# suhrig/arriba

Measured on AMD Instinct MI355X. Metric: chimeric reads/s end-to-end (BAM->fusions.tsv), synthetic, higher is better.
Workload: dtype int32

## Files before the change

### arriba_amd/csrc/device/agpu_ingest.hip

```cpp
#include <hip/hip_runtime.h>
#include <algorithm>
#include <cstring>
#include <string>
#include <vector>
#include <rocprim/rocprim.hpp>
#include "agpu_context.hpp"
#include "ingest_core.hpp"
#include "device_utils.hpp"
#include "shard_host.hpp"
#include "crc32_core.hpp"
#include "inflate_fast_core.hpp"

using namespace agpu;
namespace agpu { extern thread_local bool g_inside_ingest_finish; }

namespace {

const int BLOCK = 256;
inline unsigned int grid_for(uint64_t n, int block = BLOCK) { return (unsigned int) ((n + block - 1) / block); }

enum { IC_ACTIVE = 0, IC_MAPPED_READS = 1, IC_MISSING_HI = 2, IC_BROKEN = 3, IC_MALFORMED = 4, IC_CHIMERIC = 5, IC_COLLISION = 6, IC_MISMATCH = 7, IC_UNSORTED = 8, IC_MAX_NAME = 9,
       IC_MAX_READ_LENGTH = 10, IC_STRAND_COUNT = 11, IC_STRAND_MATCHING = 12, IC_RUNS_UNSORTED = 13, IC_QNAME_COMMA = 14, IC_COUNT = 16 };

#define HIP_CHECK(call) do { hipError_t e_ = (call); if (e_ != hipSuccess) { set_last_error(std::string(#call) + ": " + hipGetErrorString(e_)); return AGPU_ERR_DEVICE; } } while (0)
// ... 280 lines not shown
	block_tally(tally.chimeric, &counters[IC_CHIMERIC], &sums[1]);
}


__device__ FragmentName name_of(const IngestStream& in, const uint32_t* group_first, uint32_t ref, Rec& storage) {
	storage = load_record(in, group_first[ref >> 1]);
	return fragment_name(storage, hit_index_of(in, group_first[ref >> 1], storage), ref & 1);
}

__global__ void name_order_check_kernel(IngestStream in, const uint32_t* group_first, const uint32_t* order, uint64_t n, uint32_t* counters) {
	__shared__ uint32_t block_max;
	if (threadIdx.x == 0) block_max = 0;
	__syncthreads();
	const uint64_t i = blockIdx.x * (uint64_t) BLOCK + threadIdx.x;
	if (i < n) {
		Rec storage_a, storage_b;
		const FragmentName mine = name_of(in, group_first, order[i], storage_a);
		atomicMax(&block_max, name_length(mine));
		if (i > 0) {
			const FragmentName before = name_of(in, group_first, order[i - 1], storage_b);
			if (compare_names(before, mine) >= 0) atomicOr(&counters[IC_UNSORTED], 1u);
		}
	}
	__syncthreads();
	if (threadIdx.x == 0 && block_max) atomicMax(&counters[IC_MAX_NAME], block_max);
}

__global__ void run_itd_order_kernel(IngestStream in, const uint32_t* group_first, const uint8_t* valid, uint32_t first_group, uint32_t n_groups, uint32_t* counters) {
	const uint32_t g = first_group + blockIdx.x * BLOCK + threadIdx.x;
	if (g >= n_groups || g == 0 || !valid[2 * (size_t) (g - 1) + 1]) return;
	Rec storage_a, storage_b;
	const FragmentName mine = name_of(in, group_first, 2 * g, storage_b);
	const FragmentName before = name_of(in, group_first, 2 * (g - 1) + 1, storage_a);
	if (compare_names(before, mine) >= 0) atomicOr(&counters[IC_RUNS_UNSORTED], 1u);
}

__global__ void name_chunk_kernel(IngestStream in, const uint32_t* group_first, const uint32_t* order, uint64_t n, uint32_t chunk, uint64_t* keys) {
	const uint64_t i = blockIdx.x * (uint64_t) BLOCK + threadIdx.x;
	if (i >= n) return;
	Rec storage;
	keys[i] = name_chunk(name_of(in, group_first, order[i], storage), chunk);
}


__global__ void fragment_layout_kernel(IngestStream in, const uint32_t* group_first, const uint32_t* order, uint64_t n, const FragmentSizes* sizes, const uint32_t* qname_run ,
                                       uint32_t* cigar_words, uint32_t* sequence_bytes, uint32_t* name_lengths, uint32_t* new_group) {
	const uint64_t i = blockIdx.x * (uint64_t) BLOCK + threadIdx.x;
	if (i > n) return;
	if (i == n) { cigar_words[i] = 0; sequence_bytes[i] = 0; name_lengths[i] = 0; return; }
	const uint32_t ref = order[i];
	const FragmentSizes mine = sizes[ref];
	cigar_words[i] = mine.cigar_words; sequence_bytes[i] = mine.sequence_bytes; name_lengths[i] = mine.name_length;
	uint32_t differs = 0;
	if (i > 0 && qname_run != nullptr) differs = qname_run[ref >> 1] != qname_run[order[i - 1] >> 1];
	else if (i > 0) {
		const Rec a = load_record(in, group_first[ref >> 1]), b = load_record(in, group_first[order[i - 1] >> 1]);
		const uint32_t length = qname_length(a);
		differs = length != qname_length(b);
		for (uint32_t k = 0; k < length && !differs; ++k) differs = a.name[k] != b.name[k];
	}
	new_group[i] = differs;
}

__global__ void __launch_bounds__(BLOCK) AGPU_PACK_OCCUPANCY fragment_pack_kernel(IngestStream in, const uint32_t* group_first, const uint32_t* order, uint64_t n, const FragmentPlan* plain, const TandemPlan* itd,
                                                              const uint64_t* cigar_base, const uint64_t* sequence_base, const uint64_t* name_base, const uint32_t* group_id, PackTarget out, uint32_t* counters) {
	__shared__ uint32_t block_max;
	if (threadIdx.x == 0) block_max = 0;
	__syncthreads();
	const uint64_t i = blockIdx.x * (uint64_t) BLOCK + threadIdx.x;
	if (i == n) out.name_offset[n] = name_base[n];
	if (i < n) {
		const uint32_t ref = order[i], g = ref >> 1;
		const bool is_itd = ref & 1;
		Fragment3 f;
		normalize_plan(in, is_itd ? itd[g].plan : plain[g], is_itd ? &itd[g].tandem : nullptr, f);
		Rec storage;
		const FragmentName name = name_of(in, group_first, ref, storage);
		atomicMax(&block_max, write_fragment(in, f, name, i, cigar_base[i], sequence_base[i], name_base[i], group_id[i], out));
	}
	__syncthreads();
	if (threadIdx.x == 0 && block_max) atomicMax(&counters[IC_MAX_READ_LENGTH], block_max);
}

template <bool INFLATED> __global__ void __launch_bounds__(256) bgzf_crc_kernel(const uint8_t* raw, const agpu_bgzf_block* blocks, uint32_t n_blocks, const Crc32Tables* tables, unsigned int* mismatches) {
	__shared__ uint32_t slice[4][256];
	__shared__ uint32_t join[2][4][256];
	__shared__ uint32_t staged[4][CRC32_WAVE_LANES * (CRC32_ROUND_WORDS + 1)];
	for (uint32_t k = threadIdx.x; k < 4 * 256; k += 256) ((uint32_t*) slice)[k] = ((const uint32_t*) tables->slice)[k];
	for (uint32_t k = threadIdx.x; k < 2 * 4 * 256; k += 256) ((uint32_t*) join)[k] = ((const uint32_t*) tables->join)[k];
	const uint32_t wave = threadIdx.x / CRC32_WAVE_LANES, lane = threadIdx.x % CRC32_WAVE_LANES, b = blockIdx.x * 4 + wave;
	agpu_bgzf_block block;
	block.crc32 = 0; block.payload_size = 0; block.raw_offset = 0; block.payload_offset = 0;
	if (b < n_blocks) block = blocks[b];
	if (INFLATED) { block.raw_offset = block.stream_offset; block.payload_offset = 0; block.payload_size = block.isize; }
	const bool checked = b < n_blocks && block.crc32 != 0 && block.payload_size <= CRC32_VIRTUAL;
	const uint8_t* payload = raw + block.raw_offset + block.payload_offset;
	const uint32_t n = block.payload_size;
	uint32_t* mine = staged[wave];
	uint32_t c = 0;
	const bool by_chunks = checked && n >= 4;
	const uint32_t first_word = by_chunks ? (CRC32_VIRTUAL - n) / 4 : CRC32_VIRTUAL / 4;
	for (uint32_t round = 0; round < CRC32_WAVE_CHUNK / 4 / CRC32_ROUND_WORDS; ++round) {
		__syncthreads();
		for (uint32_t item = lane; item < CRC32_WAVE_LANES * CRC32_ROUND_WORDS; item += CRC32_WAVE_LANES) {
			const uint32_t chunk = item / CRC32_ROUND_WORDS, j = item % CRC32_ROUND_WORDS, w = chunk * (CRC32_WAVE_CHUNK / 4) + round * CRC32_ROUND_WORDS + j;
			mine[chunk * (CRC32_ROUND_WORDS + 1) + j] = w >= first_word ? crc32_virtual_word(payload, n, w) : 0u;
		}
		__syncthreads();
		for (uint32_t j = 0; j < CRC32_ROUND_WORDS; ++j) c = crc32_raw_step(slice, c, mine[lane * (CRC32_ROUND_WORDS + 1) + j]);
	}
	__syncthreads();
	mine[lane] = c;
	__syncthreads();
	if (lane % 8 == 0) { for (uint32_t i = 1; i < 8; ++i) c = crc32_apply(join[0], c) ^ mine[lane + i]; }
	__syncthreads();
	if (lane % 8 == 0) mine[lane] = c;
	__syncthreads();
	if (lane == 0 && checked) {
		for (uint32_t g = 1; g < 8; ++g) c = crc32_apply(join[1], c) ^ mine[8 * g];
		c ^= 0xFFFFFFFFu;
		if (n < 4) c = crc32_of_sliced(slice, payload, n);
		if (c != block.crc32) atomicAdd(mismatches, 1u);
	}
}

__global__ void shard_rebase_kernel(uint32_t* out, const uint32_t* in, uint64_t n, uint32_t base, const uint8_t* n_aln, uint32_t slot) {
	const uint64_t i = (uint64_t) blockIdx.x * blockDim.x + threadIdx.x;
	if (i < n) out[i] = in[i] + ((slot >= 3 || slot < n_aln[i]) ? base : 0u);
}
__global__ void shard_rebase_names_kernel(uint64_t* out, const uint64_t* in, uint64_t n, uint64_t base) {
	const uint64_t i = (uint64_t) blockIdx.x * blockDim.x + threadIdx.x;
	if (i < n) out[i] = in[i] + base;
}
__global__ void shard_add_coverage_kernel(uint32_t* windows, uint8_t* starts, uint8_t* ends, const uint32_t* part_windows, const uint8_t* part_starts, const uint8_t* part_ends, uint64_t n) {
	const uint64_t i = (uint64_t) blockIdx.x * blockDim.x + threadIdx.x;
	if (i < n) { windows[i] += part_windows[i]; starts[i] |= part_starts[i]; ends[i] |= part_ends[i]; }
}
__global__ void shard_add_counts_kernel(unsigned long long* counts, const unsigned long long* part, uint32_t n) {
	const uint32_t i = blockIdx.x * blockDim.x + threadIdx.x;
	if (i < n) counts[i] += part[i];
}

__global__ void packed_name_length_kernel(const uint64_t* name_offset, uint64_t n, uint32_t* longest) {
	const uint64_t i = blockIdx.x * (uint64_t) BLOCK + threadIdx.x;
	if (i < n) atomicMax(longest, (uint32_t) (name_offset[i + 1] - name_offset[i]));
}
__global__ void packed_name_chunk_kernel(const char* names, const uint64_t* name_offset, const uint32_t* order, uint64_t n, uint32_t chunk, uint64_t* keys) {
	const uint64_t i = blockIdx.x * (uint64_t) BLOCK + threadIdx.x;
	if (i >= n) return;
	const uint32_t row = order[i]; const uint64_t begin = name_offset[row]; const uint32_t length = (uint32_t) (name_offset[row + 1] - begin);
	uint64_t key = 0;
	for (uint32_t k = 0; k < 8; ++k) { const uint32_t at = 8 * chunk + k; key = key << 8 | (at < length ? (uint8_t) names[begin + at] : 0u); }
	keys[i] = key;
}
__global__ void packed_name_neighbours_kernel(const char* names, const uint64_t* name_offset, const uint32_t* order, uint64_t n, uint32_t* new_group, uint32_t* equal_names) {
	const uint64_t i = blockIdx.x * (uint64_t) BLOCK + threadIdx.x;
	if (i >= n) return;
	if (i == 0) { new_group[0] = 0; return; }
	const uint32_t a = order[i - 1], b = order[i]; const uint64_t begin_a = name_offset[a], begin_b = name_offset[b]; const uint32_t length_a = (uint32_t) (name_offset[a + 1] - begin_a), length_b = (uint32_t) (name_offset[b + 1] - begin_b);
	bool same = length_a == length_b;
	for (uint32_t k = 0; same && k < length_a; ++k) same = names[begin_a + k] == names[begin_b + k];
	if (same) atomicAdd(equal_names, 1u);
	uint32_t qname_a = length_a, qname_b = length_b;
	while (qname_a > 0 && names[begin_a + qname_a - 1] != ',') --qname_a;
	while (qname_b > 0 && names[begin_b + qname_b - 1] != ',') --qname_b;
	bool same_qname = qname_a == qname_b;
	for (uint32_t k = 0; same_qname && k < qname_a; ++k) same_qname = names[begin_a + k] == names[begin_b + k];
	new_group[i] = same_qname ? 0u : 1u;
}
__global__ void qname_run_flag_kernel(IngestStream in, uint64_t n_records, uint8_t* flags) {
	const uint64_t r = blockIdx.x * (uint64_t) BLOCK + threadIdx.x;
	if (r < n_records) flags[r] = starts_qname_run(in, (uint32_t) r) ? 1 : 0;
}
__global__ void qname_key_kernel(IngestStream in, const uint32_t* run_starts, uint64_t n_runs, uint64_t* keys) {
	const uint64_t k = blockIdx.x * (uint64_t) BLOCK + threadIdx.x;
	if (k < n_runs) qname_key128(load_record(in, run_starts[k]), keys[2 * k], keys[2 * k + 1]);
}
__global__ void qname_low_kernel(const uint64_t* keys, uint64_t n, uint64_t* low) { const uint64_t k = blockIdx.x * (uint64_t) BLOCK + threadIdx.x; if (k < n) low[k] = keys[2 * k]; }
__global__ void qname_equal_kernel(const uint64_t* low_sorted, const uint32_t* index_sorted, const uint64_t* keys, uint64_t n, uint32_t* equal) {
	const uint64_t k = blockIdx.x * (uint64_t) BLOCK + threadIdx.x;
	if (k > 0 && k < n && low_sorted[k] == low_sorted[k - 1] && keys[2 * (uint64_t) index_sorted[k] + 1] == keys[2 * (uint64_t) index_sorted[k - 1] + 1]) atomicAdd(equal, 1u);
}
__global__ void separate_name_key_kernel(const char* names, const uint64_t* name_offset, uint64_t n, uint64_t* keys) {
	const uint64_t i = blockIdx.x * (uint64_t) BLOCK + threadIdx.x;
	if (i >= n) return;
	const uint64_t begin = name_offset[i], size = name_offset[i + 1] - begin;
	keys[i] = qname_bytes_key((const uint8_t*) names + begin, size >= 2 ? (uint32_t) (size - 2) : 0u);
}
__global__ void separate_keep_kernel(const uint32_t* order, uint64_t n, const uint8_t* fbits, const uint8_t* n_aln, const uint8_t* abits_split_read, const uint8_t* abits_supplementary, uint32_t first_part, uint8_t* keep, uint32_t* inconsistent) {
	const uint64_t i = blockIdx.x * (uint64_t) BLOCK + threadIdx.x;
	if (i >= n) return;
	const uint32_t row = order[i];
	const bool of_pass_c = row < first_part, single_end = fbits[row] & FBIT_SINGLE_END;
	keep[i] = !(of_pass_c && single_end);
	if (of_pass_c && !single_end && n_aln[row] == 3 && ((abits_split_read[row] ^ abits_supplementary[row]) & ABIT_FIRST_IN_PAIR)) atomicAdd(inconsistent, 1u);
}
__global__ void iota_kernel(uint32_t* out, uint64_t n) { const uint64_t i = blockIdx.x * (uint64_t) BLOCK + threadIdx.x; if (i < n) out[i] = (uint32_t) i; }

__global__ void coverage_from_differences_kernel(const uint32_t* summed, const uint64_t* window_offset, uint32_t n_contigs, uint64_t n, uint32_t* counts, uint16_t* out) {
	const uint64_t i = blockIdx.x * (uint64_t) BLOCK + threadIdx.x;
	if (i >= n) return;
	uint32_t low = 0, high = n_contigs;
	while (high - low > 1) { const uint32_t middle = (low + high) / 2; if (window_offset[middle] <= i) low = middle; else high = middle; }
	const uint32_t count = summed[i + low];
	counts[i] = count;
	out[i] = count > 65535u ? (uint16_t) 65535 : (uint16_t) count;
// ... 256 lines not shown
			}
			if (w.known == w.enqueued && w.enqueued < 4 && (k == 0 || p.windows[k - 1].known > w.enqueued || (w.enqueued == 3 && p.windows[k - 1].enqueued == 4))) { TRY(window_step(ctx, w)); moved = true; }
		}
		while (!p.windows.empty() && p.windows.front().known == 4) { p.events.push_back(p.windows.front().readback); p.windows.pop_front(); moved = true; }
		if (moved) continue;
		if (!wait) break;
		for (size_t k = 0; k < p.windows.size(); ++k) if (p.windows[k].enqueued > p.windows[k].known) { HIP_CHECK(hipEventSynchronize(p.windows[k].readback)); break; }
	}
	return AGPU_OK;
}

int window_make(agpu_ctx* ctx, bool last) {
	IngestProgress& p = ctx->ingest_progress;
	const uint64_t size = ctx->ingest_stream_size, base = ctx->ingest_first_record;
	uint64_t segment_end = 0;
	if (last) segment_end = size > base ? (size - base + SEGMENT_BYTES - 1) / SEGMENT_BYTES : 0;
	else if (size > base + g_window_margin) segment_end = (size - base - g_window_margin) / SEGMENT_BYTES;
	if (!last && segment_end <= p.segments_done) return AGPU_OK;
	while (p.windows.size() + 2 > INGEST_WINDOW_RING) {
		IngestWindow& oldest = p.windows.front();
		if (oldest.enqueued > oldest.known) HIP_CHECK(hipEventSynchronize(oldest.readback));
		TRY(windows_advance(ctx, false));
		if (p.abandoned) return AGPU_OK;
	}
	IngestWindow w;
	w.avail = size; w.segment_begin = p.segments_done; w.segment_end = std::max(segment_end, p.segments_done); w.last = last; w.slot = p.next_slot; p.next_slot = (p.next_slot + 1) % INGEST_WINDOW_RING;
	if (!p.events.empty()) { w.readback = p.events.back(); p.events.pop_back(); } else HIP_CHECK(hipEventCreateWithFlags(&w.readback, hipEventDisableTiming));
	p.segments_done = w.segment_end; p.window_bytes = size; ++p.windows_made;
	if (ctx->ingest_pushes > 0) HIP_CHECK(hipStreamWaitEvent(p.work, ctx->piece_ready[(ctx->ingest_pushes - 1) % AGPU_PIECE_SLOTS], 0));
	p.windows.push_back(w);
	if (p.windows.size() == 1 || p.windows[p.windows.size() - 2].enqueued >= 1) TRY(window_step(ctx, p.windows.back()));
	return AGPU_OK;
}

int windows_after_push(agpu_ctx* ctx) {
	IngestProgress& p = ctx->ingest_progress;
	if (!p.on || p.abandoned) return AGPU_OK;
	TRY(windows_advance(ctx, false));
	if (!p.abandoned && ctx->ingest_stream_size - p.window_bytes >= g_window_bytes) TRY(window_make(ctx, false));
	return AGPU_OK;
}

void fill_pack_target(agpu_ctx* ctx, PackTarget& out) {
	out.n_aln = ctx->n_aln.as<uint8_t>(); out.fbits = ctx->fbits.as<uint8_t>(); out.group = ctx->group.as<uint32_t>();
	for (int k = 0; k < 3; ++k) {
		out.contig[k] = ctx->contig[k].as<uint16_t>(); out.start[k] = ctx->start[k].as<int32_t>(); out.end[k] = ctx->end[k].as<int32_t>(); out.abits[k] = ctx->abits[k].as<uint8_t>();
		out.cigar_offset[k] = ctx->cigar_offset[k].as<uint32_t>(); out.cigar_count[k] = ctx->cigar_count[k].as<uint16_t>();
	}
	out.cigar_pool = ctx->cigar_pool.as<uint32_t>();
	for (int k = 0; k < 2; ++k) { out.seq_offset[k] = ctx->seq_offset[k].as<uint32_t>(); out.seq_length[k] = ctx->seq_length[k].as<uint32_t>(); }
	out.seq_pool = ctx->seq_pool.as<uint8_t>(); out.name_offset = ctx->name_offset.as<uint64_t>(); out.row_name_offset = nullptr; out.names = ctx->names.as<char>();
}

struct BgzfPiece {
	const uint8_t* raw; const agpu_bgzf_block* blocks; uint32_t n_blocks;
	uint64_t raw_bytes, stream_bytes;
	uint8_t* target;
	uint8_t* spill;
	int lanes;
	unsigned long long* notes; uint32_t* note_count; int* status;
	int* verdict;
	unsigned int* counters;
	const Crc32Tables* crc_tables;
	hipEvent_t ready_before, ready;
};
int launch_bgzf_piece(agpu_ctx* ctx, hipStream_t pieces, bool deflated, const BgzfPiece& p) {
	const uint32_t n_blocks = p.n_blocks;
	if (deflated) {
		unsigned int* failures = p.counters + 1;
		if (p.lanes == -1) {
			KernelTimer timer(ctx, "bgzf_inflate_kernel", p.raw_bytes + p.stream_bytes, pieces);
			bgzf_inflate_kernel<<<n_blocks, 64, 0, pieces>>>(p.raw, p.blocks, p.target, p.spill, nullptr, p.verdict, failures);
		} else {
			{ KernelTimer timer(ctx, "bgzf_inflate_tokens_kernel", p.raw_bytes + p.stream_bytes, pieces);
			  #define TOKENS(LANES) bgzf_inflate_tokens_kernel<LANES><<<(n_blocks + LANES - 1) / LANES, LANES, 0, pieces>>>(p.raw, p.blocks, n_blocks, p.target, p.spill, p.notes, p.note_count, p.status, failures)
			  if (p.lanes == 16) TOKENS(16); else if (p.lanes == 24) TOKENS(24); else TOKENS(20);
			  #undef TOKENS
			}
			bgzf_inflate_kernel<<<n_blocks, 64, 0, pieces>>>(p.raw, p.blocks, p.target, p.spill, p.status, p.verdict, failures);
			{ KernelTimer timer(ctx, "bgzf_inflate_resolve_kernel", p.stream_bytes, pieces);
			  bgzf_inflate_resolve_kernel<<<(n_blocks + BLOCK / 64 - 1) / (BLOCK / 64), BLOCK, 0, pieces>>>(p.blocks, n_blocks, p.target, p.spill, p.notes, p.note_count, p.status); }
		}
	}
	else { KernelTimer timer(ctx, "bgzf_unwrap_kernel", p.raw_bytes + p.stream_bytes, pieces);
	  bgzf_unwrap_kernel<<<n_blocks, BLOCK, 0, pieces>>>(p.raw, p.blocks, p.target); }
	if (p.ready_before) HIP_CHECK(hipStreamWaitEvent(pieces, p.ready_before, 0));
	if (p.ready) HIP_CHECK(hipEventRecord(p.ready, pieces));
	if (p.crc_tables) {
		KernelTimer timer(ctx, "bgzf_crc_kernel", deflated ? p.stream_bytes : p.raw_bytes, pieces);
		if (deflated) bgzf_crc_kernel<true><<<(n_blocks + 3) / 4, 256, 0, pieces>>>(p.target, p.blocks, n_blocks, p.crc_tables, p.counters);
		else bgzf_crc_kernel<false><<<(n_blocks + 3) / 4, 256, 0, pieces>>>(p.raw, p.blocks, n_blocks, p.crc_tables, p.counters);
	}
	return AGPU_OK;
}
int upload_crc_tables(agpu_ctx* ctx) {
	if (ctx->scratch("ingest.crc_tables").ptr != nullptr) return AGPU_OK;
	ALLOC(ctx->scratch("ingest.crc_tables"), sizeof(Crc32Tables));
	static Crc32Tables tables; static bool made = false;
	if (!made) { crc32_make_tables(tables); made = true; }
	HIP_CHECK(hipMemcpy(ctx->scratch("ingest.crc_tables").ptr, &tables, sizeof(tables), hipMemcpyHostToDevice));
	return AGPU_OK;
}

}

int agpu::ingest_grow_stream(agpu_ctx* ctx, uint64_t needed) { return grow_stream(ctx, needed); }
int agpu::ingest_piece_pushed(agpu_ctx* ctx) {
	TRY(wait_for_previous_push(ctx));
	++ctx->ingest_pushes;
	return windows_after_push(ctx);
}

bool agpu::release_ingest_buffers(agpu_ctx* ctx) {
	bool released = ctx->ingest_stream.ptr != nullptr;
	ctx->ingest_stream.release(); for (int k = 0; k < AGPU_PIECE_SLOTS; ++k) ctx->ingest_raw[k].release();
	if (!ctx->ingest_part_of_sample) ctx->coverage_windows32.release();
	static const char* const temporary[] = { "ingest.record_offset", "ingest.keys", "ingest.keys_sorted", "ingest.record_bits", "ingest.sorted_records", "ingest.head", "ingest.group_start", "ingest.first_flags", "ingest.stream_rank", "ingest.group_first", "ingest.group_begin", "ingest.group_count", "ingest.plain_plans", "ingest.itd_plans",
		"ingest.valid", "ingest.sizes", "ingest.refs", "ingest.order", "ingest.order_keys", "ingest.order_keys_sorted", "ingest.cigar_words", "ingest.sequence_bytes", "ingest.name_lengths", "ingest.new_group", "ingest.cigar_base",
		"ingest.sequence_base", "ingest.name_base", "ingest.group_id", "ingest.qname_differs", "ingest.qname_run", "ingest.run_keys", "ingest.run_keys_sorted", "ingest.window_rocprim", "ingest.segment_first", "ingest.segment_end", "ingest.segment_end_before", "ingest.segment_count", "ingest.segment_base", "ingest.segment_mismatch", "ingest.rocprim", "ingest.coverage_summed", "ingest.hit_index",
		"sam.wave_count", "sam.wave_base", "sam.line_start", "sam.record_size", "sam.record_offset", "sam.rocprim", "sam.tool_text", "sam.tool_records",
		"bgzf.tool_raw", "bgzf.tool_blocks", "bgzf.tool_out", "bgzf.tool_notes", "bgzf.tool_note_count", "bgzf.tool_status", "bgzf.tool_verdict",
		"sortedbam.keys", "sortedbam.keys_sorted", "sortedbam.order", "sortedbam.sizes", "sortedbam.sizes_sorted", "sortedbam.end_flag", "sortedbam.out_offset", "sortedbam.block_first", "sortedbam.staging", "sortedbam.rocprim", "sortedbam.crc_tables",
		"sortedbam.ref_length", "sortedbam.interval_offset", "sortedbam.intervals", "sortedbam.ref_stats", "sortedbam.heads", "sortedbam.chunk_id", "sortedbam.chunk_key", "sortedbam.chunk_begin", "sortedbam.chunk_end", "sortedbam.chunk_key_sorted", "sortedbam.chunk_order", "sortedbam.chunk_out" };
	ctx->last_ingest_kept = false;
	for (size_t k = 0; k < sizeof(temporary) / sizeof(temporary[0]); ++k) { DeviceBuffer& buffer = ctx->scratch(temporary[k]); if (buffer.ptr != nullptr) released = true; buffer.release(); }
	return released;
}

extern "C" {

void* agpu_host_alloc(size_t bytes) {
	void* pointer = nullptr;
	if (hipHostMalloc(&pointer, bytes ? bytes : 16, hipHostMallocDefault) != hipSuccess) { set_last_error("hipHostMalloc failed"); return nullptr; }
	return pointer;
}
void agpu_host_free(void* pointer) { if (pointer) (void) hipHostFree(pointer); }

static int gather_rows_prepare(agpu_ctx* ctx, const uint32_t* fragments, uint64_t n, uint64_t* pool_sizes);

int agpu_ingest_begin(agpu_ctx* ctx, const agpu_ingest_config* config) {
	if (!ctx || !config) { set_last_error("null argument"); return AGPU_ERR_INVALID; }
	if (!ctx->have_annotation || !ctx->have_genome) { set_last_error("annotation and genome must be uploaded before the ingest"); return AGPU_ERR_INVALID; }
	if (config->n_contigs != ctx->genome.n_contigs) { set_last_error("the genome view on the device does not hold the contigs of the BAM header (upload it after the header was parsed)"); return AGPU_ERR_INVALID; }
	HIP_CHECK(hipSetDevice(ctx->device));
	hipStream_t s = ctx->stream;
	{ std::lock_guard<std::mutex> lock(ctx->profile_mutex); ctx->failed_launch.clear(); }
	if (!ctx->piece_stream) {
		int least = 0, greatest = 0;
		HIP_CHECK(hipDeviceGetStreamPriorityRange(&least, &greatest));
		const char* priorities = getenv("ARRIBA_STREAM_PRIORITIES");
		const bool pieces_first = priorities == nullptr || strcmp(priorities, "stages") != 0;
		HIP_CHECK(hipStreamCreateWithPriority(&ctx->piece_stream, hipStreamNonBlocking, pieces_first ? greatest : (least + greatest) / 2));
		HIP_CHECK(hipStreamCreateWithPriority(&ctx->piece_stream2, hipStreamNonBlocking, pieces_first ? greatest : (least + greatest) / 2));
		for (int k = 0; k < AGPU_PIECE_SLOTS; ++k) { HIP_CHECK(hipEventCreateWithFlags(&ctx->piece_copied[k], hipEventDisableTiming | hipEventBlockingSync));  HIP_CHECK(hipEventCreateWithFlags(&ctx->piece_ready[k], hipEventDisableTiming)); HIP_CHECK(hipEventCreateWithFlags(&ctx->piece_done[k], hipEventDisableTiming)); }
	}
	if (config->host_buffers > AGPU_PIECE_SLOTS) { set_last_error("agpu_ingest_config.host_buffers: at most 4"); return AGPU_ERR_INVALID; }
	if (config->role > AGPU_ROLE_SEPARATE_RNA || (config->role != AGPU_ROLE_WHOLE && config->part_of_sample)) { set_last_error("agpu_ingest_config.role: AGPU_ROLE_WHOLE, AGPU_ROLE_SEPARATE_CHIMERIC or AGPU_ROLE_SEPARATE_RNA, the latter two not as a part of a sample"); return AGPU_ERR_INVALID; }
	if (config->role == AGPU_ROLE_SEPARATE_RNA && !ctx->separate_adopted) { set_last_error("the main alignments of -c (AGPU_ROLE_SEPARATE_RNA) come behind agpu_separate_adopt of the separate chimeric file"); return AGPU_ERR_INVALID; }
	ctx->ingest_host_buffers = config->host_buffers < 2 ? 2 : config->host_buffers;
	ctx->last_ingest_kept = false; if (ctx->sibling) ctx->sibling->last_ingest_kept = false;
	ctx->ingest_n_targets = config->n_targets; ctx->ingest_first_record = config->first_record_offset; ctx->ingest_stream_size = 0; ctx->ingest_pushes = 0; ctx->ingest_deflated_pieces = false; ctx->ingest_sam = false;
	{ const char* knob = getenv("ARRIBA_VERIFY_CRC"); ctx->ingest_verify_crc = !(knob != nullptr && knob[0] == '0'); }
	ALLOC(ctx->scratch("ingest.crc_mismatches"), 8);
	if (ctx->ingest_verify_crc) TRY(upload_crc_tables(ctx));
	HIP_CHECK(hipMemsetAsync(ctx->scratch("ingest.crc_mismatches").ptr, 0, 8, s));
	ctx->ingest_external_duplicate_marking = config->external_duplicate_marking; ctx->ingest_max_itd_length = config->max_itd_length;
	ctx->ingest_role = config->role; ctx->ingest_part_of_sample = config->part_of_sample != 0 || config->role != AGPU_ROLE_WHOLE;
	if (config->role != AGPU_ROLE_SEPARATE_RNA) { ctx->separate_adopted = false; ctx->separate_block.release(); ctx->separate_keys.release(); ctx->separate_rows.release(); ctx->separate_n = 0; }
	ALLOC(ctx->ingest_tid_to_contig, std::max<size_t>(config->n_targets, 1) * 4);
	if (config->n_targets) HIP_CHECK(hipMemcpyAsync(ctx->ingest_tid_to_contig.ptr, config->tid_to_contig, (size_t) config->n_targets * 4, hipMemcpyHostToDevice, s));
	ctx->host_coverage_window_offset.assign(config->coverage_window_offset, config->coverage_window_offset + config->n_contigs + 1);
	const uint64_t windows = ctx->host_coverage_window_offset.back();
	ALLOC(ctx->coverage_window_offset, ((size_t) config->n_contigs + 1) * 8); ALLOC(ctx->coverage_windows32, std::max<uint64_t>(coverage_difference_slots(windows, config->n_contigs), 1) * 4); ALLOC(ctx->coverage_windows, std::max<uint64_t>(windows, 1) * 2);
	ALLOC(ctx->coverage_fragment_starts, std::max<uint64_t>(windows, 1)); ALLOC(ctx->coverage_fragment_ends, std::max<uint64_t>(windows, 1));
// ... 1022 lines not shown
```

### arriba_amd/csrc/device/crc32_core.hpp

```cpp
#ifndef AGPU_CRC32_CORE_HPP
#define AGPU_CRC32_CORE_HPP 1

#include "views.hpp"

namespace agpu {

const uint32_t CRC32_POLYNOMIAL = 0xEDB88320u;

AGPU_HD uint32_t crc32_table_entry(uint32_t i) {
	uint32_t c = i;
	for (int k = 0; k < 8; ++k) c = (c & 1u) ? (c >> 1) ^ CRC32_POLYNOMIAL : c >> 1;
	return c;
}
AGPU_HD uint32_t crc32_of(const uint32_t* table, const uint8_t* bytes, size_t n) {
	uint32_t c = 0xFFFFFFFFu;
	for (size_t i = 0; i < n; ++i) c = table[(c ^ bytes[i]) & 0xFFu] ^ (c >> 8);
	return c ^ 0xFFFFFFFFu;
}
AGPU_HD uint32_t gf2_matrix_times(const uint32_t* matrix, uint32_t vector) {
	uint32_t sum = 0;
	for (int k = 0; vector != 0; vector >>= 1, ++k) if (vector & 1u) sum ^= matrix[k];
	return sum;
}
AGPU_HD void gf2_matrix_square(uint32_t* square, const uint32_t* matrix) { for (int k = 0; k < 32; ++k) square[k] = gf2_matrix_times(matrix, matrix[k]); }
AGPU_HD uint32_t crc32_update_sliced(const uint32_t (*slice)[256], uint32_t c, const uint8_t* bytes, size_t n) {
	size_t i = 0;
	for (; i + 4 <= n; i += 4) {
		uint32_t word; __builtin_memcpy(&word, bytes + i, 4);
		c ^= word;
		c = slice[3][c & 0xFFu] ^ slice[2][(c >> 8) & 0xFFu] ^ slice[1][(c >> 16) & 0xFFu] ^ slice[0][c >> 24];
	}
	for (; i < n; ++i) c = slice[0][(c ^ bytes[i]) & 0xFFu] ^ (c >> 8);
	return c;
}
AGPU_HD uint32_t crc32_joined(uint32_t crc_a, uint32_t crc_b, uint64_t length_b) {
	if (length_b == 0) return crc_a;
	uint32_t even[32], odd[32];
	odd[0] = CRC32_POLYNOMIAL;
	uint32_t row = 1;
	for (int k = 1; k < 32; ++k) { odd[k] = row; row <<= 1; }
	gf2_matrix_square(even, odd);
	gf2_matrix_square(odd, even);
	do {
		gf2_matrix_square(even, odd);
		if (length_b & 1u) crc_a = gf2_matrix_times(even, crc_a);
		length_b >>= 1;
		if (length_b == 0) break;
		gf2_matrix_square(odd, even);
		if (length_b & 1u) crc_a = gf2_matrix_times(odd, crc_a);
		length_b >>= 1;
	} while (length_b != 0);
	return crc_a ^ crc_b;
}

const uint32_t CRC32_CHUNK = 256;

const int CRC32_ADVANCE_POWERS = 17;
const uint32_t CRC32_WAVE_CHUNK = 1024, CRC32_WAVE_LANES = 64, CRC32_VIRTUAL = CRC32_WAVE_CHUNK * CRC32_WAVE_LANES, CRC32_ROUND_WORDS = 16;
struct Crc32Tables { uint32_t slice[4][256]; uint32_t advance[CRC32_ADVANCE_POWERS][32]; uint32_t join[2][4][256]; };
AGPU_HD uint32_t crc32_apply(const uint32_t (*op)[256], uint32_t c) { return op[0][c & 0xFFu] ^ op[1][(c >> 8) & 0xFFu] ^ op[2][(c >> 16) & 0xFFu] ^ op[3][c >> 24]; }
AGPU_HD uint32_t crc32_raw_step(const uint32_t (*slice)[256], uint32_t c, uint32_t word) {
	c ^= word;
	return slice[3][c & 0xFFu] ^ slice[2][(c >> 8) & 0xFFu] ^ slice[1][(c >> 16) & 0xFFu] ^ slice[0][c >> 24];
}
AGPU_HD uint32_t crc32_virtual_word(const uint8_t* payload, uint32_t n, uint32_t w) {
	const int32_t m = (int32_t) (4 * w) - (int32_t) (CRC32_VIRTUAL - n);
	if (m + 4 <= 0) return 0;
	uint32_t word = 0;
	if (m >= 0) __builtin_memcpy(&word, payload + m, 4);
	else for (int32_t i = -m; i < 4; ++i) word |= (uint32_t) payload[m + i] << (8 * i);
	if (m < 4) for (int32_t i = 0; i < 4; ++i) if (m + i >= 0 && m + i < 4) word ^= 0xFFu << (8 * i);
	return word;
}
inline uint32_t crc32_fold_chunks(const Crc32Tables& t, const uint32_t* chunk ) {
	uint32_t group[8];
	for (uint32_t g = 0; g < 8; ++g) { uint32_t c = chunk[8 * g]; for (uint32_t i = 1; i < 8; ++i) c = crc32_apply(t.join[0], c) ^ chunk[8 * g + i]; group[g] = c; }
	uint32_t c = group[0];
	for (uint32_t g = 1; g < 8; ++g) c = crc32_apply(t.join[1], c) ^ group[g];
	return c ^ 0xFFFFFFFFu;
}
inline void crc32_make_tables(Crc32Tables& t) {
	for (uint32_t i = 0; i < 256; ++i) t.slice[0][i] = crc32_table_entry(i);
	for (int k = 1; k < 4; ++k) for (uint32_t i = 0; i < 256; ++i) t.slice[k][i] = (t.slice[k - 1][i] >> 8) ^ t.slice[0][t.slice[k - 1][i] & 0xFFu];
	uint32_t even[32], odd[32];
	odd[0] = CRC32_POLYNOMIAL;
	uint32_t row = 1;
	for (int k = 1; k < 32; ++k) { odd[k] = row; row <<= 1; }
	gf2_matrix_square(even, odd); gf2_matrix_square(odd, even);
	gf2_matrix_square(t.advance[0], odd);
	for (int k = 1; k < CRC32_ADVANCE_POWERS; ++k) gf2_matrix_square(t.advance[k], t.advance[k - 1]);
	for (int j = 0; j < 2; ++j)
		for (uint32_t b = 0; b < 4; ++b) for (uint32_t v = 0; v < 256; ++v) t.join[j][b][v] = gf2_matrix_times(t.advance[j == 0 ? 10 : 13], v << (8 * b));
}
AGPU_HD uint32_t crc32_of_sliced(const uint32_t (*slice)[256], const uint8_t* bytes, size_t n) {
	uint32_t c = 0xFFFFFFFFu;
	size_t i = 0;
	for (; i + 4 <= n; i += 4) {
		uint32_t word; __builtin_memcpy(&word, bytes + i, 4);
		c ^= word;
		c = slice[3][c & 0xFFu] ^ slice[2][(c >> 8) & 0xFFu] ^ slice[1][(c >> 16) & 0xFFu] ^ slice[0][c >> 24];
	}
	for (; i < n; ++i) c = slice[0][(c ^ bytes[i]) & 0xFFu] ^ (c >> 8);
	return c ^ 0xFFFFFFFFu;
}
AGPU_HD uint32_t crc32_joined_with(const uint32_t (*advance)[32], uint32_t crc_a, uint32_t crc_b, uint32_t length_b) {
	for (int k = 0; length_b != 0; length_b >>= 1, ++k) if (length_b & 1u) crc_a = gf2_matrix_times(advance[k], crc_a);
	return crc_a ^ crc_b;
}

}

#endif
```

Before: 58.95 million.

## Fuse BGZF unwrap copy with CRC check using 16-byte row-interleaved CRC

Result: no change. 58.87 million (-0.1%).

```diff
diff --git a/arriba_amd/csrc/device/agpu_ingest.hip b/arriba_amd/csrc/device/agpu_ingest.hip
--- a/arriba_amd/csrc/device/agpu_ingest.hip
+++ b/arriba_amd/csrc/device/agpu_ingest.hip
@@ -386,46 +386,78 @@
 	if (threadIdx.x == 0 && block_max) atomicMax(&counters[IC_MAX_READ_LENGTH], block_max);
 }
 
-template <bool INFLATED> __global__ void __launch_bounds__(256) bgzf_crc_kernel(const uint8_t* raw, const agpu_bgzf_block* blocks, uint32_t n_blocks, const Crc32Tables* tables, unsigned int* mismatches) {
-	__shared__ uint32_t slice[4][256];
-	__shared__ uint32_t join[2][4][256];
-	__shared__ uint32_t staged[4][CRC32_WAVE_LANES * (CRC32_ROUND_WORDS + 1)];
-	for (uint32_t k = threadIdx.x; k < 4 * 256; k += 256) ((uint32_t*) slice)[k] = ((const uint32_t*) tables->slice)[k];
-	for (uint32_t k = threadIdx.x; k < 2 * 4 * 256; k += 256) ((uint32_t*) join)[k] = ((const uint32_t*) tables->join)[k];
-	const uint32_t wave = threadIdx.x / CRC32_WAVE_LANES, lane = threadIdx.x % CRC32_WAVE_LANES, b = blockIdx.x * 4 + wave;
-	agpu_bgzf_block block;
-	block.crc32 = 0; block.payload_size = 0; block.raw_offset = 0; block.payload_offset = 0;
-	if (b < n_blocks) block = blocks[b];
-	if (INFLATED) { block.raw_offset = block.stream_offset; block.payload_offset = 0; block.payload_size = block.isize; }
-	const bool checked = b < n_blocks && block.crc32 != 0 && block.payload_size <= CRC32_VIRTUAL;
-	const uint8_t* payload = raw + block.raw_offset + block.payload_offset;
-	const uint32_t n = block.payload_size;
-	uint32_t* mine = staged[wave];
+const int CRC_WAVES = 4;
+__device__ __forceinline__ uint4 load_unit(const uint8_t* p) { uint4 v; __builtin_memcpy(&v, p, sizeof(v)); return v; }
+template <bool MOVE> __device__ __forceinline__ void crc_rows_body(const uint8_t* raw, const agpu_bgzf_block* blocks, uint32_t n_blocks, uint8_t* stream, const Crc32Tables* tables, unsigned int* mismatches) {
+	__shared__ __attribute__((aligned(16))) uint32_t slice16[16][256];
+	__shared__ __attribute__((aligned(16))) uint32_t row[4][256];
+	__shared__ uint32_t advance16[6][32];
+	for (uint32_t k = threadIdx.x; k < 16 * 256 / 4; k += CRC_WAVES * 64) ((uint4*) slice16)[k] = ((const uint4*) tables->slice16)[k];
+	for (uint32_t k = threadIdx.x; k < 4 * 256 / 4; k += CRC_WAVES * 64) ((uint4*) row)[k] = ((const uint4*) tables->row)[k];
+	if (threadIdx.x < 6 * 32) advance16[threadIdx.x / 32][threadIdx.x % 32] = tables->advance[4 + threadIdx.x / 32][threadIdx.x % 32];
+	__syncthreads();
+	const uint32_t lane = threadIdx.x % 64, b = blockIdx.x * CRC_WAVES + threadIdx.x / 64;
+	if (b >= n_blocks) return;
+	const agpu_bgzf_block block = blocks[b];
+	const uint32_t n = MOVE ? block.payload_size : block.isize;
+	const bool checked = block.crc32 != 0 && n <= CRC32_VIRTUAL;
+	if (!MOVE && !checked) return;
+	uint8_t* target = stream + block.stream_offset;
+	const uint8_t* source = MOVE ? raw + block.raw_offset + block.payload_offset : target;
+	const Crc32Rows r = crc32_rows_of((uint32_t) ((uintptr_t) target % CRC32_UNIT), n);
 	uint32_t c = 0;
-	const bool by_chunks = checked && n >= 4;
-	const uint32_t first_word = by_chunks ? (CRC32_VIRTUAL - n) / 4 : CRC32_VIRTUAL / 4;
-	for (uint32_t round = 0; round < CRC32_WAVE_CHUNK / 4 / CRC32_ROUND_WORDS; ++round) {
-		__syncthreads();
-		for (uint32_t item = lane; item < CRC32_WAVE_LANES * CRC32_ROUND_WORDS; item += CRC32_WAVE_LANES) {
-			const uint32_t chunk = item / CRC32_ROUND_WORDS, j = item % CRC32_ROUND_WORDS, w = chunk * (CRC32_WAVE_CHUNK / 4) + round * CRC32_ROUND_WORDS + j;
-			mine[chunk * (CRC32_ROUND_WORDS + 1) + j] = w >= first_word ? crc32_virtual_word(payload, n, w) : 0u;
-		}
-		__syncthreads();
-		for (uint32_t j = 0; j < CRC32_ROUND_WORDS; ++j) c = crc32_raw_step(slice, c, mine[lane * (CRC32_ROUND_WORDS + 1) + j]);
-	}
-	__syncthreads();
-	mine[lane] = c;
-	__syncthreads();
-	if (lane % 8 == 0) { for (uint32_t i = 1; i < 8; ++i) c = crc32_apply(join[0], c) ^ mine[lane + i]; }
-	__syncthreads();
-	if (lane % 8 == 0) mine[lane] = c;
-	__syncthreads();
-	if (lane == 0 && checked) {
-		for (uint32_t g = 1; g < 8; ++g) c = crc32_apply(join[1], c) ^ mine[8 * g];
-		c ^= 0xFFFFFFFFu;
-		if (n < 4) c = crc32_of_sliced(slice, payload, n);
+	uint4 held[3];
+	AGPU_UNROLL
+	for (uint32_t j = 0; j < 3; ++j) { held[j] = make_uint4(0, 0, 0, 0); if (64 * (j + 1) + lane < r.whole) held[j] = load_unit(source + ((size_t) CRC32_UNIT * (64 * (j + 1) + lane) - r.pad)); }
+	if (lane < r.whole) {
+		uint32_t word[4];
+		crc32_virtual_unit(source, n, r.pad, lane, word);
+		c = crc32_row_step(row, slice16, 0u, word[0], word[1], word[2], word[3]);
+		if (MOVE && (lane > 0 || r.pad == 0)) *(uint4*) (target + ((size_t) CRC32_UNIT * lane - r.pad)) = load_unit(source + ((size_t) CRC32_UNIT * lane - r.pad));
+	}
+	if (MOVE && r.whole > 0 && r.pad > 0 && lane >= r.pad && lane < CRC32_UNIT) target[lane - r.pad] = source[lane - r.pad];
+	uint32_t first = 64;
+	for (; first + 6 * 64 <= r.whole; first += 3 * 64) {
+		uint4 next[3];
+		AGPU_UNROLL for (uint32_t j = 0; j < 3; ++j) if (MOVE) *(uint4*) (target + ((size_t) CRC32_UNIT * (first + 64 * j + lane) - r.pad)) = held[j];
+		AGPU_UNROLL for (uint32_t j = 0; j < 3; ++j) next[j] = load_unit(source + ((size_t) CRC32_UNIT * (first + 64 * (j + 3) + lane) - r.pad));
+		AGPU_UNROLL for (uint32_t j = 0; j < 3; ++j) c = crc32_row_step(row, slice16, c, held[j].x, held[j].y, held[j].z, held[j].w);
+		AGPU_UNROLL for (uint32_t j = 0; j < 3; ++j) held[j] = next[j];
+	}
+	AGPU_UNROLL
+	for (uint32_t j = 0; j < 3; ++j) {
+		const uint32_t k = first + 64 * j + lane;
+		if (k < r.whole) {
+			if (MOVE) *(uint4*) (target + ((size_t) CRC32_UNIT * k - r.pad)) = held[j];
+			c = crc32_row_step(row, slice16, c, held[j].x, held[j].y, held[j].z, held[j].w);
+		}
+	}
+	for (first += 3 * 64; first < r.whole; first += 64) {
+		const uint32_t k = first + lane;
+		if (k < r.whole) {
+			const uint4 unit = load_unit(source + ((size_t) CRC32_UNIT * k - r.pad));
+			if (MOVE) *(uint4*) (target + ((size_t) CRC32_UNIT * k - r.pad)) = unit;
+			c = crc32_row_step(row, slice16, c, unit.x, unit.y, unit.z, unit.w);
+		}
+	}
+	if (MOVE && lane < r.tail) {
+		const int32_t m = (int32_t) (CRC32_UNIT * r.whole + lane) - (int32_t) r.pad;
+		if (m >= 0) target[m] = source[m];
+	}
+	if (!checked) return;
+	c = crc32_advance_units(advance16, c, crc32_units_behind(r.whole, lane));
+	for (int distance = 32; distance > 0; distance >>= 1) c ^= __shfl_xor(c, distance);
+	if (lane == 0) {
+		c = crc32_rows_tail(slice16[0], c, source, r) ^ 0xFFFFFFFFu;
+		if (n < 4) c = crc32_of_sliced(slice16, source, n);
 		if (c != block.crc32) atomicAdd(mismatches, 1u);
 	}
+}
+__global__ void __launch_bounds__(CRC_WAVES * 64) bgzf_unwrap_crc_kernel(const uint8_t* raw, const agpu_bgzf_block* blocks, uint32_t n_blocks, uint8_t* stream, const Crc32Tables* tables, unsigned int* mismatches) {
+	crc_rows_body<true>(raw, blocks, n_blocks, stream, tables, mismatches);
+}
+__global__ void __launch_bounds__(CRC_WAVES * 64) bgzf_crc_rows_kernel(const agpu_bgzf_block* blocks, uint32_t n_blocks, uint8_t* stream, const Crc32Tables* tables, unsigned int* mismatches) {
+	crc_rows_body<false>(nullptr, blocks, n_blocks, stream, tables, mismatches);
 }
 
 __global__ void shard_rebase_kernel(uint32_t* out, const uint32_t* in, uint64_t n, uint32_t base, const uint8_t* n_aln, uint32_t slot) {
@@ -848,14 +880,17 @@
 			  bgzf_inflate_resolve_kernel<<<(n_blocks + BLOCK / 64 - 1) / (BLOCK / 64), BLOCK, 0, pieces>>>(p.blocks, n_blocks, p.target, p.spill, p.notes, p.note_count, p.status); }
 		}
 	}
+	else if (p.crc_tables) {
+		KernelTimer timer(ctx, "bgzf_unwrap_crc_kernel", p.raw_bytes + p.stream_bytes, pieces);
+		bgzf_unwrap_crc_kernel<<<(n_blocks + CRC_WAVES - 1) / CRC_WAVES, CRC_WAVES * 64, 0, pieces>>>(p.raw, p.blocks, n_blocks, p.target, p.crc_tables, p.counters);
+	}
 	else { KernelTimer timer(ctx, "bgzf_unwrap_kernel", p.raw_bytes + p.stream_bytes, pieces);
 	  bgzf_unwrap_kernel<<<n_blocks, BLOCK, 0, pieces>>>(p.raw, p.blocks, p.target); }
 	if (p.ready_before) HIP_CHECK(hipStreamWaitEvent(pieces, p.ready_before, 0));
 	if (p.ready) HIP_CHECK(hipEventRecord(p.ready, pieces));
-	if (p.crc_tables) {
-		KernelTimer timer(ctx, "bgzf_crc_kernel", deflated ? p.stream_bytes : p.raw_bytes, pieces);
-		if (deflated) bgzf_crc_kernel<true><<<(n_blocks + 3) / 4, 256, 0, pieces>>>(p.target, p.blocks, n_blocks, p.crc_tables, p.counters);
-		else bgzf_crc_kernel<false><<<(n_blocks + 3) / 4, 256, 0, pieces>>>(p.raw, p.blocks, n_blocks, p.crc_tables, p.counters);
+	if (deflated && p.crc_tables) {
+		KernelTimer timer(ctx, "bgzf_crc_rows_kernel", p.stream_bytes, pieces);
+		bgzf_crc_rows_kernel<<<(n_blocks + CRC_WAVES - 1) / CRC_WAVES, CRC_WAVES * 64, 0, pieces>>>(p.blocks, n_blocks, p.target, p.crc_tables, p.counters);
 	}
 	return AGPU_OK;
 }
diff --git a/arriba_amd/csrc/device/crc32_core.hpp b/arriba_amd/csrc/device/crc32_core.hpp
--- a/arriba_amd/csrc/device/crc32_core.hpp
+++ b/arriba_amd/csrc/device/crc32_core.hpp
@@ -57,7 +57,8 @@
 
 const int CRC32_ADVANCE_POWERS = 17;
 const uint32_t CRC32_WAVE_CHUNK = 1024, CRC32_WAVE_LANES = 64, CRC32_VIRTUAL = CRC32_WAVE_CHUNK * CRC32_WAVE_LANES, CRC32_ROUND_WORDS = 16;
-struct Crc32Tables { uint32_t slice[4][256]; uint32_t advance[CRC32_ADVANCE_POWERS][32]; uint32_t join[2][4][256]; };
+const uint32_t CRC32_UNIT = 16, CRC32_ROW_BYTES = CRC32_UNIT * CRC32_WAVE_LANES;
+struct Crc32Tables { uint32_t slice[4][256]; uint32_t advance[CRC32_ADVANCE_POWERS][32]; uint32_t join[2][4][256]; uint32_t slice16[16][256]; uint32_t row[4][256]; };
 AGPU_HD uint32_t crc32_apply(const uint32_t (*op)[256], uint32_t c) { return op[0][c & 0xFFu] ^ op[1][(c >> 8) & 0xFFu] ^ op[2][(c >> 16) & 0xFFu] ^ op[3][c >> 24]; }
 AGPU_HD uint32_t crc32_raw_step(const uint32_t (*slice)[256], uint32_t c, uint32_t word) {
 	c ^= word;
@@ -79,6 +80,10 @@
 	for (uint32_t g = 1; g < 8; ++g) c = crc32_apply(t.join[1], c) ^ group[g];
 	return c ^ 0xFFFFFFFFu;
 }
+AGPU_HD uint32_t crc32_joined_with(const uint32_t (*advance)[32], uint32_t crc_a, uint32_t crc_b, uint32_t length_b) {
+	for (int k = 0; length_b != 0; length_b >>= 1, ++k) if (length_b & 1u) crc_a = gf2_matrix_times(advance[k], crc_a);
+	return crc_a ^ crc_b;
+}
 inline void crc32_make_tables(Crc32Tables& t) {
 	for (uint32_t i = 0; i < 256; ++i) t.slice[0][i] = crc32_table_entry(i);
 	for (int k = 1; k < 4; ++k) for (uint32_t i = 0; i < 256; ++i) t.slice[k][i] = (t.slice[k - 1][i] >> 8) ^ t.slice[0][t.slice[k - 1][i] & 0xFFu];
@@ -91,6 +96,9 @@
 	for (int k = 1; k < CRC32_ADVANCE_POWERS; ++k) gf2_matrix_square(t.advance[k], t.advance[k - 1]);
 	for (int j = 0; j < 2; ++j)
 		for (uint32_t b = 0; b < 4; ++b) for (uint32_t v = 0; v < 256; ++v) t.join[j][b][v] = gf2_matrix_times(t.advance[j == 0 ? 10 : 13], v << (8 * b));
+	for (uint32_t i = 0; i < 256; ++i) t.slice16[0][i] = t.slice[0][i];
+	for (int k = 1; k < 16; ++k) for (uint32_t i = 0; i < 256; ++i) t.slice16[k][i] = (t.slice16[k - 1][i] >> 8) ^ t.slice[0][t.slice16[k - 1][i] & 0xFFu];
+	for (uint32_t b = 0; b < 4; ++b) for (uint32_t v = 0; v < 256; ++v) t.row[b][v] = crc32_joined_with(t.advance, v << (8 * b), 0, CRC32_ROW_BYTES - CRC32_UNIT);
 }
 AGPU_HD uint32_t crc32_of_sliced(const uint32_t (*slice)[256], const uint8_t* bytes, size_t n) {
 	uint32_t c = 0xFFFFFFFFu;
@@ -103,9 +111,47 @@
 	for (; i < n; ++i) c = slice[0][(c ^ bytes[i]) & 0xFFu] ^ (c >> 8);
 	return c ^ 0xFFFFFFFFu;
 }
-AGPU_HD uint32_t crc32_joined_with(const uint32_t (*advance)[32], uint32_t crc_a, uint32_t crc_b, uint32_t length_b) {
-	for (int k = 0; length_b != 0; length_b >>= 1, ++k) if (length_b & 1u) crc_a = gf2_matrix_times(advance[k], crc_a);
-	return crc_a ^ crc_b;
+
+
+struct Crc32Rows { uint32_t pad, whole, tail; };
+AGPU_HD Crc32Rows crc32_rows_of(uint32_t destination_mod_16, uint32_t n) { Crc32Rows r; r.pad = destination_mod_16 % CRC32_UNIT; r.whole = (r.pad + n) / CRC32_UNIT; r.tail = (r.pad + n) % CRC32_UNIT; return r; }
+AGPU_HD void crc32_load_unit(const uint8_t* payload, uint32_t pad, uint32_t k, uint32_t word[4]) { __builtin_memcpy(word, payload + ((size_t) CRC32_UNIT * k - pad), CRC32_UNIT); }
+AGPU_HD void crc32_edge_unit(const uint8_t* payload, uint32_t n, uint32_t pad, uint32_t k, uint32_t word[4]) {
+	word[0] = word[1] = word[2] = word[3] = 0;
+	AGPU_UNROLL
+	for (uint32_t i = 0; i < CRC32_UNIT; ++i) {
+		const int32_t m = (int32_t) (CRC32_UNIT * k + i) - (int32_t) pad;
+		if (m >= 0 && m < (int32_t) n) word[i / 4] |= (uint32_t) (uint8_t) (payload[m] ^ (m < 4 ? 0xFFu : 0u)) << (8 * (i % 4));
+	}
+}
+AGPU_HD void crc32_virtual_unit(const uint8_t* payload, uint32_t n, uint32_t pad, uint32_t k, uint32_t word[4]) {
+	if (k < 2) crc32_edge_unit(payload, n, pad, k, word); else crc32_load_unit(payload, pad, k, word);
+}
+AGPU_HD uint32_t crc32_row_step(const uint32_t (*row)[256], const uint32_t (*slice16)[256], uint32_t c, uint32_t w0, uint32_t w1, uint32_t w2, uint32_t w3) {
+	w0 ^= crc32_apply(row, c);
+	return slice16[15][w0 & 0xFFu] ^ slice16[14][(w0 >> 8) & 0xFFu] ^ slice16[13][(w0 >> 16) & 0xFFu] ^ slice16[12][w0 >> 24]
+	     ^ slice16[11][w1 & 0xFFu] ^ slice16[10][(w1 >> 8) & 0xFFu] ^ slice16[9][(w1 >> 16) & 0xFFu] ^ slice16[8][w1 >> 24]
+	     ^ slice16[7][w2 & 0xFFu] ^ slice16[6][(w2 >> 8) & 0xFFu] ^ slice16[5][(w2 >> 16) & 0xFFu] ^ slice16[4][w2 >> 24]
+	     ^ slice16[3][w3 & 0xFFu] ^ slice16[2][(w3 >> 8) & 0xFFu] ^ slice16[1][(w3 >> 16) & 0xFFu] ^ slice16[0][w3 >> 24];
+}
+AGPU_HD uint32_t crc32_units_behind(uint32_t whole, uint32_t lane) { return lane < whole ? (whole - 1 - lane) % CRC32_WAVE_LANES : 0u; }
+AGPU_HD uint32_t crc32_advance_units(const uint32_t (*advance16)[32] , uint32_t c, uint32_t units) {
+	for (uint32_t bit = 0; bit < 6; ++bit) {
+		const uint32_t* matrix = advance16[bit];
+		uint32_t sum = 0;
+		AGPU_UNROLL
+		for (uint32_t k = 0; k < 32; ++k) sum ^= matrix[k] & (0u - ((c >> k) & 1u));
+		c = (units >> bit) & 1u ? sum : c;
+	}
+	return c;
+}
+AGPU_HD uint32_t crc32_rows_tail(const uint32_t* bytewise , uint32_t c, const uint8_t* payload, const Crc32Rows& r) {
+	for (uint32_t i = 0; i < r.tail; ++i) {
+		const int32_t m = (int32_t) (CRC32_UNIT * r.whole + i) - (int32_t) r.pad;
+		const uint32_t byte = m < 0 ? 0u : (uint32_t) (uint8_t) (payload[m] ^ (m < 4 ? 0xFFu : 0u));
+		c = bytewise[(c ^ byte) & 0xFFu] ^ (c >> 8);
+	}
+	return c;
 }
 
 }
```
